# iagostorch/VVC-MIP-GPU

Measured on AMD Instinct MI355X. Metric: 1080p frames/sec, full MIP mode search over all CU sizes; 1/2/4/8 GPU, higher is better.
Workload: dtype int16x2/int32

## Files before the change

vvc-mip-gpu_amd/csrc/mip_kernels.h:

```cpp
#pragma once
#include <hip/hip_runtime.h>
#include <stdint.h>

#include "mipgpu.h"

namespace mipgpu {

struct Job {
  uint32_t cost;
  uint8_t lx, ly;
  uint16_t cu;
};
struct WaveTask {
  uint8_t cls;
  uint8_t ncu;
  uint8_t q0, q1;
  uint32_t cu0;
};

constexpr int kNumClasses = 29;
constexpr int kNumBaseClasses = 17;
constexpr int kClassW[kNumClasses] = {64, 32, 32, 16, 32, 8, 16, 16, 8, 32, 4, 16, 4, 8, 8, 4, 4, 32, 16, 16, 8,
                                      4, 4, 4, 8, 8, 8, 32, 16};
constexpr int kClassH[kNumClasses] = {64, 32, 16, 32, 8, 32, 16, 8, 16, 4, 32, 4, 16, 8, 4, 8, 4, 8, 16, 8, 16,
                                      32, 16, 8, 32, 16, 16, 16, 32};
#ifndef MIP_SIX_WAVES
#define MIP_SIX_WAVES 3
#endif
constexpr int kV16 = MIP_SIX_WAVES == 1 || MIP_SIX_WAVES == 2 ? 2 : 1;
constexpr int kClassV[kNumClasses] = {4, 2, 1, 2, 1, 1, kV16, kV16, 1, 1, 2, 1, 2, 1, 1, 1, 1, 2, 4, 2, 4,
                                      2, 2, 1, 1, 1, 4, 2, 4};
constexpr bool kClassTR[kNumClasses] = {false, false, false, false, false, false, false, false, false, false, false,
                                        false, false, false, false, false, false, false, false, false, false,
                                        true, true, true, true, true, true, false, false};
constexpr int kClassVariant[kNumClasses] = {-1, -1, 27, 28, 17, -1, 18, 19, 20, -1, -1, -1, -1, -1, -1, -1, -1,
                                            -1, -1, -1, -1, -1, -1, -1, -1, 26, -1, -1, -1};
constexpr int kClassTransposed[kNumBaseClasses] = {-1, -1, -1, -1, 24, -1, -1, 25, -1, 21, -1, 22, -1, -1, 23, -1, -1};
constexpr int size_class(int w, int h) {
  for (int i = 0; i < kNumBaseClasses; i++)
    if (kClassW[i] == w && kClassH[i] == h) return i;
  return -1;
}
constexpr int class_size_id(int w, int h) { return (w == 4 && h == 4) ? 0 : ((w == 4 || h == 4 || (w == 8 && h == 8)) ? 1 : 2); }
constexpr int class_slots(int cls) { return 64 / ((kClassW[cls] / 4) * kClassV[cls]); }

struct SearchArgs {
  const uint16_t *orig;
  const uint16_t *refs;
  int32_t *cost;
  uint8_t *best_mode;
  int32_t *best_cost;
  uint32_t *split_acc;
  const uint16_t *dfill;
  const int *dfill_begin;
  int32_t *sad;
  int32_t *satd;
  const WaveTask *tasks;
  const Job *jobs;
  const int *list_begin;
  const uint32_t *fill;
  const int *fill_begin;
  const uint8_t *ctu_var;
  const uint4 *tables;
  int width, height;
  int ctu_cols, nctus;
  int ctu0, nrange;
  int slices;
  uint32_t *queue;
  uint32_t nitems;
  const uint32_t *order;
  uint32_t nframes;
  uint32_t chunks;
  uint64_t *wave_clock;
  uint32_t *status;
  uint32_t *const *frame_status;
  int check_refs;
  uint32_t nonempty;
};
constexpr int kStatusOrig = 0, kStatusRefs = 1, kStatusWords = 4;
constexpr uint32_t kAbove10Bits = 0xfc00fc00u;
constexpr int kClockSlots = 128;
constexpr int kQueueChunks = 8;
constexpr int kQueueWords = 16;
constexpr int kMaxCtuVariants = 255;

constexpr float kAccInitS2 = 0.5f - 1024.0f;
constexpr int kWeightRows = 768, kWeightRowOffS1 = 384, kWeightRowOffS0 = 512;
constexpr int kCtabRows = 384 + 4;
constexpr int kTableBytes = kWeightRows * 16 + kCtabRows * 4;

struct FixupCu {
  uint32_t ctu;
  uint16_t cu;
  uint8_t shape;
  uint8_t pad;
};

struct BestArgs {
  const int32_t *cost;
  uint8_t *best_mode;
  int32_t *best_cost;
  int total_cus;
  int k;
};
constexpr int kMaxBestK = 32;

struct FilterArgs {
  const uint16_t *in;
  uint16_t *out;
  int width, height, nframes;
  int filter;
  int kernel_idx;
};

constexpr int kSearchWaves = MIP_SIX_WAVES == 1 || MIP_SIX_WAVES == 3 ? 12 : 8, kWideWaves = 16;
int search_resident_groups(bool alt_refs, bool wide);
#if !defined(MIP_FOUR_WAVE_TWIN) || !MIP_FOUR_WAVE_TWIN
int search_resident_groups_four(bool alt_refs, bool wide);
#endif
hipError_t launch_search(const SearchArgs &a, int nframes, bool alt_refs, int resident, bool wide, hipStream_t s,
                         hipEvent_t done = nullptr);
#if !defined(MIP_FOUR_WAVE_TWIN) || !MIP_FOUR_WAVE_TWIN
hipError_t launch_search_four(const SearchArgs &a, int nframes, bool alt_refs, int resident, bool wide, hipStream_t s,
                         hipEvent_t done = nullptr);
#endif
hipError_t launch_best_modes(const BestArgs &a, hipStream_t s);
struct SplitArgs {
  const uint16_t *split;
  const int *split_begin;
  const uint8_t *ctu_var;
  uint8_t *best_mode;
  int32_t *best_cost;
  int nctus, ctu0, nrange, max_split;
  uint32_t *acc;
};
hipError_t launch_dec_split(const SplitArgs &a, int nframes, bool init, hipStream_t s);
hipError_t launch_filter(const FilterArgs &a, hipStream_t s);
hipError_t launch_copy(const void *src, void *dst, size_t bytes, hipStream_t s);
struct CopyPiece {
  const uint8_t *src;
  uint8_t *dst;
  uint64_t bytes;
};
constexpr int kMaxCopyPieces = 64;
struct CopyPieces {
  CopyPiece p[kMaxCopyPieces];
  int n;
};
hipError_t launch_gather_copy(const CopyPieces &a, hipStream_t s);
hipError_t launch_fixup(const SearchArgs &a, const FixupCu *cus, int n, int nframes, hipStream_t s);

struct PredictArgs {
  const uint16_t *refs;
  const mip_pred_item *items;
  long long n;
  const uint8_t *unavail;
  const uint32_t *geo;
  uint16_t *out;
  long long out_samples;
  uint32_t *skipped;
  int width, height, ctu_cols, nctus, nframes;
  int refs_vec;
};
hipError_t launch_predict(const PredictArgs &a, hipStream_t s);

}
```

vvc-mip-gpu_amd/csrc/mip_search.hip:

```cpp
#include <algorithm>
#include <cstdlib>
#include <type_traits>
#include <utility>

#include <hip/hip_ext.h>

#ifndef MIP_FOUR_WAVE_TWIN
#define MIP_FOUR_WAVE_TWIN 0
#endif
#if MIP_FOUR_WAVE_TWIN
#define launch_search launch_search_four
#define search_resident_groups search_resident_groups_four
#define search_lds_bytes search_lds_bytes_four
#endif

#include "mip_kernels.h"
#include "mip_tables.h"

namespace mipgpu {
namespace {

typedef short __attribute__((ext_vector_type(2))) s2;
typedef unsigned short __attribute__((ext_vector_type(2))) u2;
typedef _Float16 __attribute__((ext_vector_type(2))) h2;
typedef _Float16 __attribute__((ext_vector_type(4))) h4;
typedef float __attribute__((ext_vector_type(4))) f4;

[[maybe_unused]] __constant__ mip_shape_desc c_shapes[MIP_NUM_SHAPES] = MIP_SHAPE_TABLE;
struct ShapeStarts {
  uint16_t v[MIP_NUM_SHAPES + 1];
};
constexpr mip_shape_desc kShapesC[MIP_NUM_SHAPES] = MIP_SHAPE_TABLE;
constexpr ShapeStarts make_shape_starts() {
  ShapeStarts st{};
  for (int i = 0; i < MIP_NUM_SHAPES; i++) st.v[i + 1] = (uint16_t)(st.v[i] + kShapesC[i].ncu);
  return st;
}
static_assert(make_shape_starts().v[MIP_NUM_SHAPES] == MIP_CUS_PER_CTU, "shape table");
[[maybe_unused]] __constant__ ShapeStarts c_shape_start = make_shape_starts();

#ifndef MIP_PREFETCH_MIN_ITEMS
#define MIP_PREFETCH_MIN_ITEMS 32
#endif
#ifndef MIP_PF_BATCH
#define MIP_PF_BATCH 10
#endif
#ifndef MIP_PHASEA_BATCH_NCS
#define MIP_PHASEA_BATCH_NCS 2
#endif
#ifndef MIP_ACC_PAIR
#define MIP_ACC_PAIR 1
#endif
#ifndef MIP_UV2_UNROLL
#define MIP_UV2_UNROLL 2
#endif
#ifndef MIP_WIN_UNROLL
#define MIP_WIN_UNROLL 2
#endif
#ifndef MIP_PAIR_BLOCKS
#define MIP_PAIR_BLOCKS 1
#endif
#ifndef MIP_PRIO_BALANCE
#define MIP_PRIO_BALANCE 0
#endif
#ifndef MIP_ONLY_CLASS
#define MIP_ONLY_CLASS -1
#endif
#ifndef MIP_SKIP_CLASSES
#define MIP_SKIP_CLASSES 0
#endif

constexpr int kPitch = 68;
constexpr int kColOff = 4;
constexpr int kTileElems = (65 * kPitch + 7) / 8 * 8;
constexpr int kLatRowPitch = kPitch, kLatColPitch = 66;
constexpr int kLatElems = (16 * kLatRowPitch + 16 * kLatColPitch + 7) / 8 * 8;
constexpr int kEntryBytes = 16;
constexpr int kCuTableBytes = 64 * kEntryBytes;
#ifndef MIP_SCRATCH_WORDS
#define MIP_SCRATCH_WORDS \
  (MIP_SIX_WAVES == 1 ? 1152 : (MIP_SIX_WAVES == 2 ? 1144 : (MIP_SIX_WAVES == 3 ? 768 : 1280)))
#endif
constexpr bool kSpanChunks = MIP_SIX_WAVES == 3;
constexpr int kScratchWords = MIP_SCRATCH_WORDS;
constexpr int kWaveBytes = kCuTableBytes + kScratchWords * 4;
constexpr int kWaveStride = kWaveBytes;
constexpr int kZeroBytes = 7 * 8 * kEntryBytes + 16;
constexpr int kUnavailable = 0x7fffffff;

constexpr uint32_t kBiasD[2][4] = {{15345, 1023, 3069, 1023}, {7161, 1023, 3069, 1023}};
constexpr uint32_t kBiasP[4] = {32736, 24552, 16368, 16368};
constexpr uint32_t kBiasQ = 8184;
constexpr uint32_t splat32(uint32_t v) { return v | v << 16; }
constexpr uint32_t bias_word(int y, int x) { return kBiasD[y & 1][x & 3] | kBiasD[y & 1][(x + 1) & 3] << 16; }

__device__ __forceinline__ int tidx(int x, int y) { return (y + 1) * kPitch + x + kColOff; }
__device__ __forceinline__ s2 as_s2(uint32_t v) { return __builtin_bit_cast(s2, v); }
__device__ __forceinline__ u2 as_u2(s2 v) { return __builtin_bit_cast(u2, v); }
__device__ __forceinline__ s2 as_s2(u2 v) { return __builtin_bit_cast(s2, v); }
__device__ __forceinline__ s2 splat(int v) { return s2{(short)v, (short)v}; }
__device__ __forceinline__ s2 smax(s2 a, s2 b) { return __builtin_elementwise_max(a, b); }

constexpr int ilog2c(int v) { return v <= 1 ? 0 : 1 + ilog2c(v / 2); }

__device__ __forceinline__ s2 avg_round(s2 a, s2 b) {
  const uint32_t t = __builtin_bit_cast(uint32_t, a) + __builtin_bit_cast(uint32_t, b) + 0x00010001u;
  return __builtin_bit_cast(s2, __builtin_bit_cast(u2, t) >> (u2){1, 1});
}

template <class F, int... I>
__device__ __forceinline__ void static_for_impl(F &f, std::integer_sequence<int, I...>) {
  (f(std::integral_constant<int, I>{}), ...);
}
template <int N, class F>
__device__ __forceinline__ void static_for(F &&f) {
  static_for_impl(f, std::make_integer_sequence<int, N>{});
}

template <int O>
__device__ __forceinline__ u2 pk_mad_c(u2 a, u2 c) {
  if constexpr (O == 1) {
    return a + c;
  } else {
    u2 d;
    asm("v_pk_mad_u16 %0, %1, %2, %3 op_sel_hi:[1,0,1]" : "=v"(d) : "v"(a), "i"(O), "v"(c));
    return d;
  }
}
template <int O, int C>
__device__ __forceinline__ u2 pk_mad_cc(u2 a) {
  u2 d;
  asm("v_pk_mad_u16 %0, %1, %2, %3 op_sel_hi:[1,0,0]" : "=v"(d) : "v"(a), "i"(O), "i"(C));
  return d;
}

__device__ __forceinline__ void wave_lds_sync() {
  __builtin_amdgcn_fence(__ATOMIC_RELEASE, "wavefront");
  __builtin_amdgcn_wave_barrier();
  __builtin_amdgcn_fence(__ATOMIC_ACQUIRE, "wavefront");
}

template <int W, int H, int VP = kClassV[size_class(W, H)]>
struct Geo {
  static constexpr int SID = class_size_id(W, H);
  static constexpr int R = SID == 2 ? 8 : 4;
  static constexpr int RBS = SID == 0 ? 2 : 4;
  static constexpr int NOUT = R * R;
  static constexpr int UH = W / R, UV = H / R;
  static constexpr int LH = ilog2c(UH), LV = ilog2c(UV);
  static constexpr int S = W / 4;
  static constexpr int V = VP;
  static constexpr int SLOTS = 64 / (S * V);
  static constexpr int KV = R / V;
  static constexpr int CROWS = UH != 1 ? (kSpanChunks && 64 / (S * V) * (R * (R + 1) + 1) > kScratchWords ? R / 2 : R)
                               : 64 / (S * V) * (NOUT + 4) <= kScratchWords ? R
                               : !kSpanChunks ? (SID == 2 ? R / 2 : R)
                               : 64 / (S * V) * (NOUT / 2 + 4) > kScratchWords ? R / 4 : R / 2;
  static constexpr bool CHUNKED = CROWS < R;
  static constexpr int NCH = R / CROWS;
  static constexpr int CPOS = CROWS * R;
  static constexpr bool PAD = UH > 1;
  static constexpr int RP = PAD ? R + 1 : R;
  static constexpr int PITCH = UH == 1 ? (SLOTS * (CPOS + 4) <= kScratchWords ? CPOS + 4 : CPOS) : CROWS * RP + 1;
  static constexpr int WBASE = SID == 2 ? 0 : (SID == 1 ? kWeightRowOffS1 : kWeightRowOffS0);
  static constexpr int MODES = SID == 2 ? 6 : (SID == 1 ? 8 : 16);
  static_assert(SLOTS * S * V == 64, "lanes");
  static_assert(SLOTS * PITCH <= kScratchWords, "scratch");
  static_assert(V == 1 || (!CHUNKED && SID != 0 && (UV >= 4 || KV % (4 / UV) == 0)), "row parts");
  static_assert(!CHUNKED || (CROWS >= 2 && (kSpanChunks || (SID == 2 && NCH == 2))), "chunks");
};

template <bool LAT>
struct RefTile {
  const uint16_t *t;
  template <int PH>
  __device__ __forceinline__ int top(int x, int y) const {
    return LAT ? t[((y + 1) >> 2) * kLatRowPitch + x + kColOff] : t[tidx(x, y)] - (int)kBiasD[1][PH];
  }
  __device__ __forceinline__ uint2 top4(int x, int y) const {
    const uint2 v = *reinterpret_cast<const uint2 *>(t + (LAT ? ((y + 1) >> 2) * kLatRowPitch + x + kColOff : tidx(x, y)));
    return LAT ? v : make_uint2(v.x - bias_word(3, 0), v.y - bias_word(3, 2));
  }
  __device__ __forceinline__ int left(int x, int y) const {
    return LAT ? t[16 * kLatRowPitch + ((x + 1) >> 2) * kLatColPitch + y + 1] : t[tidx(x, y)] - (int)kBiasD[0][3];
  }
  template <int PH>
  __device__ __forceinline__ int left_ph(int x, int y) const { return left(x, y); }
};

template <bool LAT>
struct RefTileT {
  RefTile<LAT> r;
  template <int PH>
  __device__ __forceinline__ int top(int x, int y) const { return r.left(y, x); }
  __device__ __forceinline__ uint2 top4(int x, int y) const {
    return make_uint2((uint32_t)r.left(y, x) | (uint32_t)r.left(y, x + 1) << 16,
                      (uint32_t)r.left(y, x + 2) | (uint32_t)r.left(y, x + 3) << 16);
  }
  template <int PH>
  __device__ __forceinline__ int left_ph(int x, int y) const { return r.template top<PH>(y, x); }
  __device__ __forceinline__ int left(int x, int y) const {
    const int ph = y & 3;
    return ph == 0 ? left_ph<0>(x, y) : ph == 1 ? left_ph<1>(x, y) : ph == 2 ? left_ph<2>(x, y) : left_ph<3>(x, y);
  }
};

__device__ __forceinline__ uint2 lds_row4(const uint16_t *tile, int x, int y) {
  return *reinterpret_cast<const uint2 *>(tile + tidx(x, y));
}

struct CuPos {
  int lx, ly;
  bool top, left;
  int padT, padL;
};

template <bool TR, class RT>
__device__ __forceinline__ CuPos cu_pos(const Job &j, int fx0, int fy0, const RT &rt) {
  CuPos c;
  c.lx = TR ? j.ly : j.lx;
  c.ly = TR ? j.lx : j.ly;
  c.top = (TR ? fx0 : fy0) + c.ly > 0;
  c.left = (TR ? fy0 : fx0) + c.lx > 0;
  c.padT = c.left ? rt.template left_ph<0>(c.lx - 1, c.ly) : 512;
  c.padL = c.top ? rt.template top<0>(c.lx, c.ly - 1) : 512;
  return c;
}

template <int W, int H, class RT>
__device__ __forceinline__ void write_inputs(const CuPos &c, const RT &rt, uint8_t *entry) {
  using G = Geo<W, H>;
  constexpr int dfT = W / G::RBS, l2T = ilog2c(dfT), rndT = dfT > 1 ? dfT / 2 : 0;
  constexpr int dfL = H / G::RBS, l2L = ilog2c(dfL), rndL = dfL > 1 ? dfL / 2 : 0;
  uint32_t redT[G::RBS], redL[G::RBS];
  static_for<G::RBS>([&](auto i_c) {
    constexpr int i = decltype(i_c)::value;
    uint32_t s = 0;
    if constexpr (dfT >= 4) {
#pragma unroll
      for (int t = 0; t < dfT; t += 4) {
        const uint2 v = rt.top4(c.lx + i * dfT + t, c.ly - 1);
        s += (v.x & 0xffff) + (v.x >> 16) + (v.y & 0xffff) + (v.y >> 16);
      }
    } else {
      static_for<dfT>([&](auto t_c) {
        constexpr int off = i * dfT + decltype(t_c)::value;
        s += rt.template top<off & 3>(c.lx + off, c.ly - 1);
      });
    }
    redT[i] = c.top ? (s + rndT) >> l2T : c.padT;
    uint32_t l = 0;
    static_for<dfL>([&](auto t_c) {
      constexpr int off = i * dfL + decltype(t_c)::value;
      l += rt.template left_ph<off & 3>(c.lx - 1, c.ly + off);
    });
    redL[i] = c.left ? (l + rndL) >> l2L : c.padL;
  });
  constexpr uint32_t kBias = 0x64006400u;
  uint4 e;
  if constexpr (G::RBS == 4) {
    e = make_uint4(redT[0] | redT[1] << 16, redT[2] | redT[3] << 16, redL[0] | redL[1] << 16, redL[2] | redL[3] << 16);
  } else {
    const uint32_t t01 = redT[0] | redT[1] << 16, l01 = redL[0] | redL[1] << 16;
    e = make_uint4(t01, l01, l01, t01);
  }
  e.x |= kBias;
  e.y |= kBias;
  e.z |= kBias;
  e.w |= kBias;
  *reinterpret_cast<uint4 *>(entry) = e;
}

struct BlockAcc {
  uint32_t t[16];
  uint32_t pos;
};

__device__ __forceinline__ uint32_t as_u32(s2 v) { return __builtin_bit_cast(uint32_t, v); }
__device__ __forceinline__ uint32_t as_u32(u2 v) { return __builtin_bit_cast(uint32_t, v); }
__device__ __forceinline__ u2 as_u2(uint32_t v) { return __builtin_bit_cast(u2, v); }

template <int I>
__device__ __forceinline__ void block_row(BlockAcc &b, const s2 (&prow)[4], uint2 orow) {
  constexpr const uint32_t *B = kBiasD[I & 1];
  const s2 o01 = as_s2(orow.x), o23 = as_s2(orow.y);
  const uint32_t d0 = as_u32(s2{o01.x, o01.x} - prow[0]), d1 = as_u32(s2{o01.y, o01.y} - prow[1]);
  const uint32_t d2 = as_u32(s2{o23.x, o23.x} - prow[2]), d3 = as_u32(s2{o23.y, o23.y} - prow[3]);
  const uint32_t p0 = as_u32(__builtin_elementwise_sub_sat(as_u2(d0), (u2){(unsigned short)B[0], (unsigned short)B[0]}));
  const uint32_t p1 = as_u32(__builtin_elementwise_sub_sat(as_u2(d1), (u2){(unsigned short)B[1], (unsigned short)B[1]}));
  const uint32_t p2 = as_u32(__builtin_elementwise_sub_sat(as_u2(d2), (u2){(unsigned short)B[2], (unsigned short)B[2]}));
  const uint32_t p3 = as_u32(__builtin_elementwise_sub_sat(as_u2(d3), (u2){(unsigned short)B[3], (unsigned short)B[3]}));
  b.pos = I == 0 ? p0 + p1 + p2 + p3 : b.pos + p0 + p1 + p2 + p3;
  const uint32_t s0 = d0 + d1, s1 = d0 - d1, s2_ = d2 + d3, s3 = d2 - d3;
  b.t[4 * I + 0] = s0 + s2_;
  b.t[4 * I + 1] = s1 + s3;
  b.t[4 * I + 2] = s0 - s2_;
  b.t[4 * I + 3] = s1 - s3;
}

template <uint32_t BETA>
__device__ __forceinline__ uint32_t fold_pair(uint32_t a, uint32_t b) {
  static_assert(2 * BETA < 65536, "bias");
  const u2 mx = __builtin_elementwise_max(as_u2(a), as_u2(b)), mn = __builtin_elementwise_min(as_u2(a), as_u2(b));
  const uint32_t ng = splat32(2 * BETA) - as_u32(mn);
  return as_u32(__builtin_elementwise_max(mx, as_u2(ng))) - splat32(BETA);
}

__device__ __forceinline__ void block_finish(const BlockAcc &b, u2 &sad, u2 &satd) {
  uint32_t T = 0, m0 = 0;
  s2 dc = splat(0);
  static_for<4>([&](auto c_c) {
    constexpr int c = decltype(c_c)::value;
    const uint32_t u0 = b.t[c] + b.t[4 + c], u1 = b.t[c] - b.t[4 + c];
    const uint32_t u2_ = b.t[8 + c] + b.t[12 + c], u3 = b.t[8 + c] - b.t[12 + c];
    T += fold_pair<kBiasQ>(u1, u3);
    if constexpr (c == 0) {
      m0 = fold_pair<kBiasP[0]>(u0, u2_);
      dc = as_s2(u0) - as_s2(splat32(2 * kBiasP[0]) - u2_);
    } else {
      T += fold_pair<kBiasP[c]>(u0, u2_);
    }
  });
  const s2 adc = smax(dc, splat(0) - dc);
  const uint32_t U = m0 + m0 - as_u32(adc) + as_u32(as_u2(adc) >> (u2){2, 2});
  satd = as_u2(T + as_u32(as_u2(U + 0x00010001u) >> (u2){1, 1}));
  sad = as_u2(as_s2(b.pos + b.pos) - dc);
}

struct PairAcc {
  uint32_t sad0 = 0, sad1 = 0;
  uint32_t t0 = 0, t1 = 0;
};

template <int I>
__device__ __forceinline__ void residual_row(const s2 (&prow)[4], uint2 orow, uint32_t (&d)[4]) {
  const s2 o01 = as_s2(orow.x), o23 = as_s2(orow.y);
  d[0] = as_u32(s2{o01.x, o01.x} - prow[0]);
  d[1] = as_u32(s2{o01.y, o01.y} - prow[1]);
  d[2] = as_u32(s2{o23.x, o23.x} - prow[2]);
  d[3] = as_u32(s2{o23.y, o23.y} - prow[3]);
}
// ... 70 lines not shown
    satd0 = __builtin_amdgcn_udot2(satd, (u2){1, 0}, satd0, false);
    satd1 = __builtin_amdgcn_udot2(satd, (u2){0, 1}, satd1, false);
  }
  __device__ __forceinline__ void flush() {}
#endif
};

struct PackedAcc {
  uint32_t sad = 0, satd = 0;
  __device__ __forceinline__ void add(u2 s, u2 t) {
    sad += as_u32(s);
    satd += as_u32(t);
  }
};

struct OrigT {
  uint32_t v[4];
};

struct BlockAccTr {
  uint32_t t[16];
  uint32_t pos;
};

template <int I>
__device__ __forceinline__ void residual_row(const s2 (&prow)[4], const OrigT &o, uint32_t (&d)[4]) {
#pragma unroll
  for (int c = 0; c < 4; c++) d[c] = as_u32(s2{(short)o.v[c], (short)o.v[c]} - prow[c]);
}

template <int I>
__device__ __forceinline__ void block_row(BlockAccTr &b, const s2 (&prow)[4], const OrigT &o) {
  uint32_t d[4];
  residual_row<I>(prow, o, d);
  uint32_t p = 0;
  static_for<4>([&](auto c_c) {
    constexpr int c = decltype(c_c)::value;
    constexpr unsigned short B = (unsigned short)kBiasD[c & 1][I];
    p += as_u32(__builtin_elementwise_sub_sat(as_u2(d[c]), (u2){B, B}));
    b.t[4 * I + c] = d[c];
  });
  b.pos = I == 0 ? p : b.pos + p;
}

__device__ __forceinline__ void rows_transform_tr(const uint32_t (&raw)[16], uint32_t (&t)[16]) {
#pragma unroll
  for (int r = 0; r < 4; r++) {
    const uint32_t e0 = raw[r], e1 = raw[4 + r], e2 = raw[8 + r], e3 = raw[12 + r];
    const uint32_t s0 = e0 + e1, s1 = e0 - e1, s2_ = e2 + e3, s3 = e2 - e3;
    t[4 * r + 0] = s0 + s2_;
    t[4 * r + 1] = s1 + s3;
    t[4 * r + 2] = s0 - s2_;
    t[4 * r + 3] = s1 - s3;
  }
}

__device__ __forceinline__ void block_finish(const BlockAccTr &b, u2 &sad, u2 &satd) {
  BlockAcc r;
  rows_transform_tr(b.t, r.t);
  r.pos = b.pos;
  block_finish(r, sad, satd);
}

template <int I>
__device__ __forceinline__ void pair_row_tr(const uint32_t *dA, const uint32_t (&dB)[4], uint32_t (&t0)[16],
                                            uint32_t (&t1)[16], PairAcc &acc) {
  static_for<4>([&](auto c_c) {
    constexpr int c = decltype(c_c)::value;
    const uint32_t m0 = __builtin_amdgcn_perm(dB[c], dA[c], 0x05040100u);
    const uint32_t m1 = __builtin_amdgcn_perm(dB[c], dA[c], 0x07060302u);
    acc.sad0 = __builtin_amdgcn_sad_u16(m0, splat32(kBiasD[c & 1][I]), acc.sad0);
    acc.sad1 = __builtin_amdgcn_sad_u16(m1, splat32(kBiasD[c & 1][I]), acc.sad1);
    t0[4 * I + c] = m0;
    t1[4 * I + c] = m1;
  });
}

__device__ __forceinline__ uint32_t pair_finish_tr(const uint32_t (&raw)[16], uint32_t T) {
  uint32_t t[16];
  rows_transform_tr(raw, t);
  return pair_finish(t, T);
}

template <int R, int RP = R>
struct Red {
  static constexpr int OFF = RP > R ? 1 : 0;
  const uint32_t *p;
  int k0;
  static __device__ __forceinline__ s2 clip(uint32_t v) {
    return __builtin_bit_cast(s2, __builtin_elementwise_min(__builtin_bit_cast(u2, v), (u2){1023, 1023}));
  }
  __device__ __forceinline__ s2 operator()(int k, int kx) const { return clip(p[(k + k0) * RP + kx + OFF]); }
  __device__ __forceinline__ void row4(int k, int kx, s2 (&out)[4]) const {
    static_assert(RP == R, "row4 reads unpadded rows");
    const uint4 v = *reinterpret_cast<const uint4 *>(p + (k + k0) * R + kx);
    out[0] = clip(v.x);
    out[1] = clip(v.y);
    out[2] = clip(v.z);
    out[3] = clip(v.w);
  }
};

template <int W, int H, class RED>
__device__ __forceinline__ void anchor_row(const RED &red, int k, int x0, s2 (&a)[4]) {
  using G = Geo<W, H>;
  if constexpr (G::UH == 1) {
    red.row4(k, x0, a);
  } else if constexpr (G::UH == 2) {
    const int kx = x0 >> 1;
    const s2 r0 = red(k, kx), r1 = red(k, kx + 1);
    const s2 before = red(k, kx - 1);
    a[0] = avg_round(before, r0);
    a[1] = r0;
    a[2] = avg_round(r0, r1);
    a[3] = r1;
  } else {
    const int kx = x0 >> G::LH;
    const s2 after = red(k, kx);
    const s2 before = red(k, kx - 1);
    const uint32_t delta = as_u32(after) - as_u32(before);
    const u2 base = pk_mad_cc<G::UH, G::UH / 2>(as_u2(before));
    uint32_t n = as_u32(base);
    if constexpr (G::UH == 8) {
      const u2 hdelta = as_u2(after - before);
      const uint32_t o0 = splat32(x0 & (G::UH - 1));
      u2 base0;
      asm("v_pk_mad_u16 %0, %1, %2, %3" : "=v"(base0) : "v"(hdelta), "v"(o0), "v"(base));
      n = as_u32(base0);
    }
    static_for<4>([&](auto oc) {
      constexpr int c = decltype(oc)::value;
      if constexpr (G::UH == 4 && c == 3) {
        a[c] = after;
      } else {
        n += delta;
        a[c] = as_s2(as_u2(n) >> (u2){G::LH, G::LH});
      }
    });
  }
}

template <int H>
struct OrigRows {
  static constexpr bool TR = false;
  using Block = BlockAcc;
  static constexpr bool CACHED = H <= 4;
  uint2 r[CACHED ? H : 1];
  const uint16_t *row0;
  __device__ __forceinline__ void load(const uint16_t *t, int xx, int yy) {
    row0 = t + tidx(xx, yy);
    if constexpr (CACHED) {
#pragma unroll
      for (int i = 0; i < H; i++) r[i] = lds_row4(t, xx, yy + i);
    }
  }
  __device__ __forceinline__ uint2 operator()(int i) const {
    if constexpr (CACHED) return r[i];
    else return *reinterpret_cast<const uint2 *>(row0 + i * kPitch);
  }
};

template <int H>
struct OrigRowsT {
  static constexpr bool TR = true;
  using Block = BlockAccTr;
  const uint16_t *tile;
  int x, y;
  __device__ __forceinline__ void load(const uint16_t *t, int xx, int yy) {
    tile = t;
    x = xx;
    y = yy;
  }
  __device__ __forceinline__ OrigT operator()(int i) const {
// ... 315 lines not shown
  uint8_t *wave;
  int ctu, frame;
  int fx0, fy0;
};

__device__ __forceinline__ uint32_t floor_sat(float f) { return (uint32_t)f; }

template <int W, int H, int V, bool TR>
__device__ __forceinline__ void phase_a(const Ctx &x, int lane, int ncu, int q, int chunk) {
  using G = Geo<W, H, V>;
  const int r = lane & 15, h = lane >> 4;
  const int m0 = TR ? 2 * q - G::MODES : 2 * q;
  constexpr bool HALF = G::CHUNKED && G::SID != 2;
  constexpr bool TR2 = TR && G::SID == 2 && G::CHUNKED && G::CROWS == 2;
  const int jrow = TR2 ? 8 * (r >> 1) + (r & 1) : (G::SID == 2 && TR) ? 8 * (r >> 2) + (r & 3) : r;
  const uint8_t *abase = x.w + ((G::WBASE + (m0 + (h >> 1)) * G::NOUT + jrow) * 8 + 4 * (h & 1)) * 2;
  const bool bsel = (h >> 1) == (r & 1);
  const uint8_t *bbase = bsel ? x.wave + (r >> 1) * kEntryBytes + 8 * ((h & 1) ^ (TR ? 1 : 0)) : x.zero;
  f4 cin;
  if constexpr (G::SID == 2) {
    cin = *reinterpret_cast<const f4 *>(reinterpret_cast<const float *>(x.w + kWeightRows * 16) + 384);
  } else {
    const float *ct = reinterpret_cast<const float *>(x.w + kWeightRows * 16) + (G::WBASE - kWeightRowOffS1);
    cin = *reinterpret_cast<const f4 *>(ct + (m0 + (r & 1)) * G::NOUT + 4 * h);
  }
  constexpr int NCS = (G::SLOTS + 7) / 8;
  const int ncs_run = __builtin_amdgcn_readfirstlane((ncu + 7) >> 3);
  constexpr int NRB = HALF ? 1 : G::CPOS / 16;
  constexpr int PSTEP = TR ? G::RP : 1;
  const int pos0 = TR2 ? 2 * h : TR ? h + G::PAD : (G::PAD ? (4 * h / G::R) * G::RP + (4 * h) % G::R + 1 : 4 * h);
  uint8_t *lane_dst = x.wave + kCuTableBytes + ((r >> 1) * G::PITCH + pos0) * 4 + 2 * (r & 1);
#pragma unroll
  for (int rb = 0; rb < NRB; rb++) {
    int jofs, pofs;
    if constexpr (TR2) {
      jofs = 2 * chunk;
      pofs = 0;
    } else if constexpr (G::SID == 2) {
      const int rbg = G::CHUNKED ? NRB * chunk + rb : rb;
      const int cofs = G::CHUNKED ? G::CPOS * chunk : 0;
      const int crow = G::CHUNKED ? G::CROWS * chunk * G::RP : 0;
      if constexpr (!TR) {
        jofs = 16 * rbg;
        pofs = G::PAD ? 2 * rbg * G::RP - crow : 16 * rbg - cofs;
      } else {
        const int cc = rbg >> 1, rr = rbg & 1;
        jofs = 32 * rr + 4 * cc;
        pofs = G::PAD ? 4 * cc * G::RP + 4 * rr - crow : 32 * cc + 4 * rr - cofs;
      }
    } else {
      jofs = 0;
      pofs = HALF ? -8 * chunk : 0;
    }
    const h4 av = *reinterpret_cast<const h4 *>(abase + jofs * 16);
    constexpr bool BATCH_B = NRB == 1 && NCS >= MIP_PHASEA_BATCH_NCS;
    h4 bvs[BATCH_B ? NCS : 1];
    if constexpr (BATCH_B) {
#pragma unroll
      for (int cs = 0; cs < NCS; cs++) bvs[cs] = *reinterpret_cast<const h4 *>(bbase + cs * 8 * kEntryBytes);
    }
#pragma unroll
    for (int cs = 0; cs < NCS; cs++) {
      if (cs > 0 && cs >= ncs_run) break;
      const h4 bv = BATCH_B ? bvs[BATCH_B ? cs : 0] : *reinterpret_cast<const h4 *>(bbase + cs * 8 * kEntryBytes);
      const f4 d = __builtin_amdgcn_mfma_f32_16x16x16f16(av, bv, cin, 0, 0, 0);
      if ((G::SLOTS % 8 == 0 || 8 * cs + (r >> 1) < ncu) && (!HALF || TR || (h >> 1) == chunk)) {
        uint8_t *dst = lane_dst + (pofs + 8 * cs * G::PITCH) * 4;
        static_for<4>([&](auto i_c) {
          constexpr int i = decltype(i_c)::value;
          constexpr int off = TR2 ? (i & 1) * G::R + (i >> 1) : i * PSTEP;
          if (!(HALF && TR) || (i >> 1) == chunk) {
            const uint32_t v = floor_sat(d[i]);
            *reinterpret_cast<uint16_t *>(dst + off * 4) = (uint16_t)v;
          }
        });
      }
    }
  }
}

template <int W, int H, int V, bool TR>
__device__ __forceinline__ void phase_a_half(const Ctx &x, int lane, int q, int chunk) {
  using G = Geo<W, H, V>;
  static_assert(G::CHUNKED && G::SID != 2 && G::SLOTS == 64 && G::CROWS == 2 && !G::PAD && G::PITCH >= 8, "half chunks");
  const int r = lane & 15, h = lane >> 4;
  const int m0 = TR ? 2 * q - G::MODES : 2 * q;
  auto jout = [&](int p) { return TR ? 4 * (p & 3) + 2 * chunk + (p >> 2) : 8 * chunk + p; };
  auto pos_of_row = [](int row) { return ((row >> 1) >> 1) + 4 * ((row >> 1) & 1); };
  const uint8_t *aptr = h < 2 ? x.w + ((G::WBASE + (m0 + (r & 1)) * G::NOUT + jout(pos_of_row(r))) * 8 + 4 * h) * 2
                              : x.zero;
  const h4 av = *reinterpret_cast<const h4 *>(aptr);
  const uint8_t *bbase = x.wave + r * kEntryBytes + 8 * ((h & 1) ^ (TR ? 1 : 0));
  const float *ct = reinterpret_cast<const float *>(x.w + kWeightRows * 16) + (G::WBASE - kWeightRowOffS1);
  f4 cin;
  static_for<4>([&](auto i_c) {
    constexpr int i = decltype(i_c)::value;
    cin[i] = ct[(m0 + (i & 1)) * G::NOUT + jout(h + 4 * (i >> 1))];
  });
  h4 bvs[4];
#pragma unroll
  for (int cs = 0; cs < 4; cs++) bvs[cs] = *reinterpret_cast<const h4 *>(bbase + cs * 16 * kEntryBytes);
  uint8_t *lane_dst = x.wave + kCuTableBytes + (r * G::PITCH + h) * 4;
#pragma unroll
  for (int cs = 0; cs < 4; cs++) {
    const f4 d = __builtin_amdgcn_mfma_f32_16x16x16f16(av, bvs[cs], cin, 0, 0, 0);
    uint8_t *dst = lane_dst + 16 * cs * G::PITCH * 4;
    static_for<4>([&](auto i_c) {
      constexpr int i = decltype(i_c)::value;
      typedef __attribute__((address_space(3))) volatile uint16_t lds_u16;
      *(lds_u16 *)(dst + 16 * (i >> 1) + 2 * (i & 1)) = (uint16_t)floor_sat(d[i]);
    });
  }
}

template <int W, int H, int V>
__device__ __forceinline__ void phase_a(const Ctx &x, int lane, int ncu, int q, int chunk) {
  using G = Geo<W, H, V>;
  if constexpr (G::CHUNKED && G::SID != 2) {
    if (q >= G::MODES / 2) phase_a_half<W, H, V, true>(x, lane, q, chunk);
    else phase_a_half<W, H, V, false>(x, lane, q, chunk);
  } else {
    if (q >= Geo<W, H>::MODES / 2) phase_a<W, H, V, true>(x, lane, ncu, q, chunk);
    else phase_a<W, H, V, false>(x, lane, ncu, q, chunk);
  }
}

template <int N>
__device__ __forceinline__ uint32_t group_sum(uint32_t v) {
  if constexpr (N >= 2) v += (uint32_t)__builtin_amdgcn_update_dpp(0, (int)v, 0x111, 0xf, 0xf, true);
  if constexpr (N >= 4) v += (uint32_t)__builtin_amdgcn_update_dpp(0, (int)v, 0x112, 0xf, 0xf, true);
  if constexpr (N >= 8) v += (uint32_t)__builtin_amdgcn_update_dpp(0, (int)v, 0x114, 0xf, 0xf, true);
  if constexpr (N >= 16) v += (uint32_t)__builtin_amdgcn_update_dpp(0, (int)v, 0x118, 0xf, 0xf, true);
  if constexpr (N >= 32) v += (uint32_t)__builtin_amdgcn_update_dpp(0, (int)v, 0x142, 0xa, 0xf, false);
  if constexpr (N >= 64) v += (uint32_t)__builtin_amdgcn_update_dpp(0, (int)v, 0x143, 0xc, 0xf, false);
  return v;
}

#ifndef MIP_PIN_SUMS
#define MIP_PIN_SUMS 1
#endif
__device__ __forceinline__ uint32_t pin_sum(uint32_t v) {
#if MIP_PIN_SUMS
  asm volatile("; pin" : "+v"(v));
#endif
  return v;
}

#ifndef MIP_COST_STORE_AUX
#define MIP_COST_STORE_AUX 0
#endif
struct CtuRows {
  __amdgpu_buffer_rsrc_t r;
  __device__ __forceinline__ explicit CtuRows(int32_t *ctu_block) {
    r = __builtin_amdgcn_make_buffer_rsrc(ctu_block, 0, MIP_COSTS_PER_CTU * 4, 0x00020000);
  }
  __device__ __forceinline__ void store(uint32_t cu_ofs, int mq, int v0, int v1) const {
    typedef unsigned int v2u __attribute__((ext_vector_type(2)));
    __builtin_amdgcn_raw_buffer_store_b64((v2u){(unsigned)v0, (unsigned)v1}, r, (int)cu_ofs, mq * 4, MIP_COST_STORE_AUX);
  }
};

__device__ __forceinline__ int opaque(int v) {
  asm volatile("; opaque" : "+v"(v));
  return v;
}

template <bool TR, bool LAT>
struct ViewOf {
  using type = RefTile<LAT>;
  static __device__ __forceinline__ type make(const RefTile<LAT> &r) { return r; }
};
template <bool LAT>
struct ViewOf<true, LAT> {
  using type = RefTileT<LAT>;
  static __device__ __forceinline__ type make(const RefTile<LAT> &r) { return RefTileT<LAT>{r}; }
};

template <int W, int H, int V, bool LAT, bool DEC, bool TR = false>
__device__ __forceinline__ void run_task(const Ctx &x, const RefTile<LAT> &rt_tile, const WaveTask &task, int lane_in) {
  using G = Geo<W, H, V>;
  const typename ViewOf<TR, LAT>::type rt = ViewOf<TR, LAT>::make(rt_tile);
  const int lane = opaque(lane_in);
  const SearchArgs &a = *x.a;
  const int ncu = task.ncu;
  const Job *jobs = a.jobs + task.cu0;
  const int slot = lane / (G::S * G::V), sub = lane % (G::S * G::V);
  const int v = sub / G::S, sx = sub % G::S, x0 = 4 * sx;
  const bool active = slot < ncu;
  const int cs = min(slot, ncu - 1);
  const Job job = jobs[cs];
  const CuPos c = cu_pos<TR>(job, x.fx0, x.fy0, rt);

  if (lane < ncu) {
    const Job jb = jobs[lane];
    const CuPos cj = cu_pos<TR>(jb, x.fx0, x.fy0, rt);
    write_inputs<W, H>(cj, rt, x.wave + lane * kEntryBytes);
  }
  std::conditional_t<TR, OrigRowsT<H>, OrigRows<H>> orig;
  orig.load(x.org, c.lx + x0, c.ly);
  const size_t ctu_row = ((size_t)x.frame * a.nctus + x.ctu) * MIP_COSTS_PER_CTU;
  const uint32_t cu_ofs = (uint32_t)job.cost * 4;
  const CtuRows rows_cost(a.cost ? a.cost + ctu_row : nullptr), rows_sad(a.sad ? a.sad + ctu_row : nullptr),
      rows_satd(a.satd ? a.satd + ctu_row : nullptr);
  const uint32_t *mine = reinterpret_cast<const uint32_t *>(x.wave + kCuTableBytes) + cs * G::PITCH;
  const Red<G::R, G::RP> red{mine, 0};
  s2 top[4];
  {
    const uint2 tv = rt.top4(c.lx + x0, c.ly - 1);
    const int t4[4] = {(int)(tv.x & 0xffff), (int)(tv.x >> 16), (int)(tv.y & 0xffff), (int)(tv.y >> 16)};
#pragma unroll
    for (int cc = 0; cc < 4; cc++) top[cc] = splat(c.top ? t4[cc] : c.padT);
  }
  constexpr int NLV = (G::R + G::S * G::V - 1) / (G::S * G::V);
  uint32_t lvs[G::PAD && G::CHUNKED ? NLV : 1];
  uint32_t *lcol = reinterpret_cast<uint32_t *>(x.wave + kCuTableBytes) + cs * G::PITCH;
  auto write_left = [&](int chunk) {
#pragma unroll
    for (int j = 0; j < NLV; j++) {
      const int k = sub + j * G::S * G::V;
      if (active && k < G::R && k / G::CROWS == chunk) lcol[(k - chunk * G::CROWS) * G::RP] = lvs[j];
    }
  };
  if constexpr (G::PAD && G::CHUNKED) {
#pragma unroll
    for (int j = 0; j < NLV; j++) {
      const int k = sub + j * G::S * G::V;
      const uint32_t lv = k < G::R && c.left ? rt.left(c.lx - 1, c.ly + k * G::UV + G::UV - 1) : c.padL;
      lvs[j] = lv | lv << 16;
    }
    write_left(0);
  } else if constexpr (G::PAD) {
    for (int k = sub; k < G::R; k += G::S * G::V) {
      const uint32_t lv = c.left ? rt.left(c.lx - 1, c.ly + k * G::UV + G::UV - 1) : c.padL;
      if (active) lcol[k * G::RP] = lv | lv << 16;
    }
  }
  wave_lds_sync();

  uint32_t best = 0xffffffffu;
  constexpr bool PAIRED = MIP_PAIR_BLOCKS && kPaired<W, H, V>;
#pragma unroll 1
  for (int q = task.q0; q < task.q1; q++) {
    std::conditional_t<PAIRED, PairAcc, std::conditional_t<(W * H <= 32), PackedAcc, Acc>> acc;
    s2 prev[4];
#pragma unroll
    for (int cc = 0; cc < 4; cc++) prev[cc] = top[cc];
    phase_a<W, H, V>(x, lane, ncu, q, 0);
    if constexpr (G::PAD && G::CHUNKED) {
      if (q > task.q0) write_left(0);
    }
    wave_lds_sync();
    if constexpr (kSpanChunks && G::CHUNKED) {
      auto sw = [&](int c) {
        wave_lds_sync();
        phase_a<W, H, V>(x, lane, ncu, q, c);
        if constexpr (G::PAD) write_left(c);
        wave_lds_sync();
      };
      if constexpr (G::SID == 0) {
        walk_4x4_chunked<W, H, V>(orig, red, sw, acc);
      } else {
        static_assert(PAIRED, "chunked classes walk block pairs");
        walk_pairs_chunked<W, H, V>(orig, red, x0, prev, acc, sw);
      }
    } else if constexpr (PAIRED && G::CHUNKED) {
      walk_pairs<W, H, V>(orig, red, x0, 0, prev, acc);
      wave_lds_sync();
      phase_a<W, H, V>(x, lane, ncu, q, 1);
      wave_lds_sync();
      const Red<G::R, G::RP> red_hi{mine, -4};
      walk_pairs<W, H, V>(orig, red_hi, x0, 4, prev, acc);
    } else if constexpr (PAIRED) {
      const int k0 = G::V > 1 ? v * G::KV : 0;
      if constexpr (G::V > 1) {
        if (k0 > 0) anchor_row<W, H>(red, k0 - 1, x0, prev);
      }
      walk_pairs<W, H, V>(orig, red, x0, k0, prev, acc);
    } else if constexpr (G::CHUNKED) {
      walk_strip<W, H, V>(orig, red, x0, 0, 4, prev, acc);
      wave_lds_sync();
      phase_a<W, H, V>(x, lane, ncu, q, 1);
      wave_lds_sync();
      const Red<G::R, G::RP> red_hi{mine, -4};
      walk_strip<W, H, V>(orig, red_hi, x0, 4, 8, prev, acc);
    } else if constexpr (G::SID == 0) {
      walk_strip<W, H, V>(orig, red, x0, 0, 4, prev, acc);
    } else {
      const int k0 = G::V > 1 ? v * G::KV : 0;
// ... 308 lines not shown
    if (b && s1.valid(k)) v1[k] = s1.load(k);
  }
  uint32_t bits0 = 0, bits1 = 0;
#pragma unroll
  for (int k = 0; k < N; k++) {
    if (s0.valid(k)) {
      bits0 |= v0[k].x | v0[k].y;
      s0.store(dst0, k, v0[k]);
    }
    if (b && s1.valid(k)) {
      bits1 |= v1[k].x | v1[k].y;
      s1.store(dst1, k, v1[k]);
    }
  }
  flag_above_10_bits(bits0, a, f0, kStatusOrig);
  flag_above_10_bits(bits1, a, f1, kStatusOrig);
}

template <bool DEC>
__device__ __forceinline__ void pair_loop(const SearchArgs &a, uint16_t *org_buf, const uint8_t *w, const uint8_t *zero,
                                          uint8_t *waves, uint32_t *counters, int wave, int lane) {
  const uint32_t ne = a.nonempty, npairs = (ne + 1) / 2;
  for (;;) {
    if (threadIdx.x == 0) {
      counters[0] = 0;
      counters[1] = atomicAdd(a.queue, 1u);
    }
    __syncthreads();
    const uint32_t p = counters[1];
    if (p >= npairs) break;
    const uint32_t i0 = p, i1 = ne - 1 - p;
    const bool two = i1 != i0;
    const ItemPos p0(a, i0), p1(a, i1);
    const int vq0 = a.ctu_var[p0.ctu] * 4 + p0.quad, vq1 = a.ctu_var[p1.ctu] * 4 + p1.quad;
    const int l0 = vq0 * a.slices + p0.slice, l1 = vq1 * a.slices + p1.slice;
    const int tb0 = a.list_begin[l0], n0 = a.list_begin[l0 + 1] - tb0;
    const int tb1 = a.list_begin[l1], n1 = two ? a.list_begin[l1 + 1] - tb1 : 0;
    fill_unavailable<DEC>(a, p0.frame, p0.ctu, vq0, p0.slice);
    if (two) fill_unavailable<DEC>(a, p1.frame, p1.ctu, vq1, p1.slice);
    for (uint32_t e = ne + p; e < a.nitems; e += npairs) {
      const ItemPos pe(a, e);
      fill_unavailable<DEC>(a, pe.frame, pe.ctu, a.ctu_var[pe.ctu] * 4 + pe.quad, pe.slice);
    }
    uint16_t *org0 = org_buf, *org1 = org_buf + kTileElems;
    stage_tiles2<64 * kWideWaves>(org0, a.orig + (size_t)p0.frame * a.width * a.height, p0.fx0, p0.fy0, org1,
                                  a.orig + (size_t)p1.frame * a.width * a.height, p1.fx0, p1.fy0, two, a.width,
                                  a.height, a, p0.frame, p1.frame);
    __syncthreads();
    uint64_t *clk0 = a.wave_clock ? a.wave_clock + (size_t)i0 * kClockSlots : nullptr;
    uint64_t *clk1 = a.wave_clock && two ? a.wave_clock + (size_t)i1 * kClockSlots : nullptr;
    if (clk0 && threadIdx.x == 0) {
      stamp_item_start(clk0);
      if (clk1) stamp_item_start(clk1);
    }
    const int m = n0 < n1 ? n0 : n1;
    for (;;) {
      uint32_t tn = 0;
      if (lane == 0) tn = atomicAdd(counters, 1u);
      const int t = (int)__builtin_amdgcn_readfirstlane(tn);
      if (t >= n0 + n1) break;
      const bool second = t < 2 * m ? (t & 1) != 0 : n1 > n0;
      const int k = t < 2 * m ? t >> 1 : t - m;
      const uint64_t c0 = clk0 ? __builtin_readcyclecounter() : 0;
      const WaveTask task = a.tasks[(second ? tb1 : tb0) + k];
      const Ctx x{&a, second ? org1 : org0, second ? org1 : org0, w, zero, waves + wave * kWaveStride,
                  second ? p1.ctu : p0.ctu, second ? p1.frame : p0.frame, second ? p1.fx0 : p0.fx0,
                  second ? p1.fy0 : p0.fy0};
      const RefTile<false> rt{x.ref};
      dispatch_task<false, DEC>(x, rt, task, lane);
      uint64_t *clk = second ? clk1 : clk0;
      if (clk && lane == 0) {
        if (k < kClockSlots - 3) clk[k] = __builtin_readcyclecounter() - c0;
        atomicMax(reinterpret_cast<unsigned long long *>(clk + kClockSlots - 2),
                  (unsigned long long)__builtin_amdgcn_s_memrealtime());
      }
    }
    __syncthreads();
  }
}

#ifndef MIP_WAVES_PER_EU
#define MIP_WAVES_PER_EU (MIP_SIX_WAVES ? 6 : 4)
#endif
#ifndef MIP_TABLES_GLOBAL
#define MIP_TABLES_GLOBAL 0
#endif
constexpr bool kTablesInLds = (!MIP_SIX_WAVES || MIP_SIX_WAVES == 3) && !MIP_TABLES_GLOBAL;
#ifndef MIP_S6_PF
#define MIP_S6_PF 1
#endif
#define MIP_PF_KERNEL (!MIP_SIX_WAVES || (MIP_SIX_WAVES == 3 && MIP_S6_PF))
constexpr bool kPrefetchKernel = MIP_PF_KERNEL;
template <bool ALT, bool DEC, bool PF_, int NW>
__global__ __launch_bounds__(64 * NW, NW == kWideWaves ? 4 : MIP_WAVES_PER_EU) void mip_search_kernel(SearchArgs a) {
  constexpr bool PF = PF_ && !ALT && NW == kSearchWaves && kPrefetchKernel;
  extern __shared__ __attribute__((aligned(16))) uint8_t smem[];
  uint16_t *org_buf = reinterpret_cast<uint16_t *>(smem);
  uint16_t *lattice = org_buf + kOrgTiles<ALT, PF, NW> * kTileElems;
  uint8_t *tab = smem + (kOrgTiles<ALT, PF, NW> * kTileElems + (ALT ? kLatElems : 0)) * 2;
  uint8_t *zero = tab + (kTablesInLds ? kTableBytes : 0);
  uint8_t *waves = zero + kZeroBytes;
  uint32_t *counters = reinterpret_cast<uint32_t *>(waves + NW * kWaveStride);
  const uint8_t *w = kTablesInLds ? tab : reinterpret_cast<const uint8_t *>(a.tables);

  if constexpr (kTablesInLds)
    for (int i = threadIdx.x; i < kTableBytes / 16; i += blockDim.x)
      reinterpret_cast<uint4 *>(tab)[i] = a.tables[i];
  for (int i = threadIdx.x; i < kZeroBytes / 16; i += blockDim.x)
    reinterpret_cast<uint4 *>(zero)[i] = make_uint4(0, 0, 0, 0);
  const int wave = __builtin_amdgcn_readfirstlane(threadIdx.x >> 6), lane = threadIdx.x & 63;

  if (NW == kWideWaves && !ALT && !PF && a.nonempty > 0) {
    pair_loop<DEC>(a, org_buf, w, zero, waves, counters, wave, lane);
  } else {
  if (threadIdx.x < kCounterWords) counters[threadIdx.x] = threadIdx.x == 2 && PF ? kTakeItem : 0u;
  __syncthreads();
  if (!PF) {
    if (threadIdx.x == 0) counters[2] = take_item(a, counters + 8);
    __syncthreads();
  }
  int par = 0;
  for (;;) {
    uint32_t *next_task = counters + 4 * par, *finished = next_task + 1;
    uint32_t item = next_task[2];
    bool staged = PF;
    if (PF && item == kTakeItem) {
      if (threadIdx.x == 0) next_task[3] = take_item(a, counters + 8);
      __syncthreads();
      item = next_task[3];
      staged = false;
    }
    if (item >= a.nitems) break;
    const ItemPos ip(a, item);
    const int ctu = ip.ctu, frame = ip.frame, slice = ip.slice, quad = ip.quad, fx0 = ip.fx0, fy0 = ip.fy0;
    const size_t fofs = (size_t)frame * a.width * a.height;
    const int var = a.ctu_var[ctu];
    const int vq = var * 4 + quad, list = vq * a.slices + slice;
    const int tbase = a.list_begin[list], ntasks = a.list_begin[list + 1] - tbase;
    uint16_t *org = org_buf + (PF ? par * kTileElems : 0);
    uint16_t *ref = ALT ? lattice : org;

    fill_unavailable<DEC>(a, frame, ctu, vq, slice);
    if (ntasks > 0) {
      if (!PF || !staged) {
        stage_tile<64 * NW>(org, a.orig + fofs, a.width, a.height, fx0, fy0, a, frame);
        if (ALT) stage_lattice<64 * NW>(ref, a.refs + fofs, a.width, a.height, fx0, fy0, a.check_refs != 0, a, frame);
        __syncthreads();
      }

      const Ctx x{&a, org, ref, w, zero, waves + wave * kWaveStride, ctu, frame, fx0, fy0};
      const RefTile<ALT> rt{ref};
      uint64_t *clk = a.wave_clock ? a.wave_clock + (size_t)item * kClockSlots : nullptr;
      if (clk && threadIdx.x == 0) stamp_item_start(clk);
      for (;;) {
        uint32_t tn = 0;
        if (lane == 0) tn = atomicAdd(next_task, 1u);
        const int t = (int)__builtin_amdgcn_readfirstlane(tn);
        if (t >= ntasks) break;
#if MIP_PRIO_BALANCE
        {
          const int rem4 = 4 * (ntasks - t);
          if (rem4 > 3 * ntasks) __builtin_amdgcn_s_setprio(3);
          else if (rem4 > 2 * ntasks) __builtin_amdgcn_s_setprio(2);
          else if (rem4 > ntasks) __builtin_amdgcn_s_setprio(1);
          else __builtin_amdgcn_s_setprio(0);
        }
#endif
        const uint64_t c0 = clk ? __builtin_readcyclecounter() : 0;
        const WaveTask task = a.tasks[tbase + t];
        dispatch_task<ALT, DEC>(x, rt, task, lane);
        if (clk && lane == 0 && t < kClockSlots - 3) clk[t] = __builtin_readcyclecounter() - c0;
      }
      if (clk && lane == 0) atomicMax(reinterpret_cast<unsigned long long *>(clk + kClockSlots - 2),
                                      (unsigned long long)__builtin_amdgcn_s_memrealtime());
    }
    if (PF) {
      uint32_t *nxt = counters + 4 * (par ^ 1);
      uint32_t r = 0;
      if (lane == 0) r = atomicAdd(finished, 1u);
      if (__builtin_amdgcn_readfirstlane(r) == 0) {
        uint32_t n = kTakeItem;
        if (lane == 0 && far_from_end(a, item)) n = take_item(a, counters + 8);
        const uint32_t nitem = __builtin_amdgcn_readfirstlane(n);
        if (nitem < a.nitems) {
          const ItemPos np(a, nitem);
          const uint16_t *nframe = a.orig + (size_t)np.frame * a.width * a.height;
          uint16_t *dst = org_buf + (par ^ 1) * kTileElems;
          const WindowStager<64> st(nframe, a.width, a.height, np.fx0, np.fy0, lane);
          constexpr int NL = WindowStager<64>::N, NB = MIP_PF_BATCH;
          uint32_t bits = 0;
#pragma unroll
          for (int k0 = 0; k0 < NL; k0 += NB) {
// ... 229 lines not shown
```

Baseline: 7877.

## Convert MIP phase-A MFMA outputs with packed normalized u16 conversion

Phase-A MFMA results are now converted with cvt_pknorm_u16 into packed 32-bit stores instead of four separate floor/saturate scalar u16 LDS stores. To make that exact, the input bias and accumulator init are rescaled, the size-0 bias table is prescaled while staged into LDS, and the reduced-sample clip becomes a shift. The half-zero B operand layout is also changed so A loads are unconditional and the unused half reads zeros from a shared zero region. This relies on careful float scaling to keep the results bit-exact, and it adds work to the LDS table staging.

Result: no change. 7949, median of 6 (+0.9%).

```diff
diff --git a/vvc-mip-gpu_amd/csrc/mip_kernels.h b/vvc-mip-gpu_amd/csrc/mip_kernels.h
--- a/vvc-mip-gpu_amd/csrc/mip_kernels.h
+++ b/vvc-mip-gpu_amd/csrc/mip_kernels.h
@@ -88,6 +88,8 @@
 constexpr int kWeightRows = 768, kWeightRowOffS1 = 384, kWeightRowOffS0 = 512;
 constexpr int kCtabRows = 384 + 4;
 constexpr int kTableBytes = kWeightRows * 16 + kCtabRows * 4;
+constexpr int kPkScaleLog2 = -10, kPkOffsetLog2 = -17;
+constexpr uint32_t kPkInputBias = 0x3c00;
 
 struct FixupCu {
   uint32_t ctu;
diff --git a/vvc-mip-gpu_amd/csrc/mip_search.hip b/vvc-mip-gpu_amd/csrc/mip_search.hip
--- a/vvc-mip-gpu_amd/csrc/mip_search.hip
+++ b/vvc-mip-gpu_amd/csrc/mip_search.hip
@@ -85,7 +85,7 @@
 constexpr int kScratchWords = MIP_SCRATCH_WORDS;
 constexpr int kWaveBytes = kCuTableBytes + kScratchWords * 4;
 constexpr int kWaveStride = kWaveBytes;
-constexpr int kZeroBytes = 7 * 8 * kEntryBytes + 16;
+constexpr int kZeroBytes = 7 * 8 * kEntryBytes + 16 + 16;
 constexpr int kUnavailable = 0x7fffffff;
 
 constexpr uint32_t kBiasD[2][4] = {{15345, 1023, 3069, 1023}, {7161, 1023, 3069, 1023}};
@@ -170,6 +170,28 @@
   static_assert(!CHUNKED || (CROWS >= 2 && (kSpanChunks || (SID == 2 && NCH == 2))), "chunks");
 };
 
+#ifndef MIP_PK_CONVERT
+#define MIP_PK_CONVERT 1
+#endif
+#ifndef MIP_HALF_ZERO_B
+#define MIP_HALF_ZERO_B 1
+#endif
+#ifndef MIP_DENSE_8XH
+#define MIP_DENSE_8XH 0
+#endif
+template <int W, int H, int V>
+constexpr bool kHalfA = Geo<W, H, V>::CHUNKED &&
+                        (Geo<W, H, V>::SID != 2 || (MIP_DENSE_8XH && MIP_PK_CONVERT && kSpanChunks && Geo<W, H, V>::UH == 1 &&
+                                                    Geo<W, H, V>::CROWS == 2 && Geo<W, H, V>::SLOTS % 16 == 0));
+template <int W, int H, int V>
+constexpr bool kPackedA = MIP_PK_CONVERT && kHalfA<W, H, V>;
+#ifndef MIP_TABLES_GLOBAL
+#define MIP_TABLES_GLOBAL 0
+#endif
+constexpr bool kTablesInLds = (!MIP_SIX_WAVES || MIP_SIX_WAVES == 3) && !MIP_TABLES_GLOBAL;
+constexpr bool kPkStagedS0 = kPackedA<4, 4, 1> && kTablesInLds;
+constexpr float kPkScale = 1.0f / (float)(1 << -kPkScaleLog2), kPkOffset = 1.0f / (float)(1 << -kPkOffsetLog2);
+
 template <bool LAT>
 struct RefTile {
   const uint16_t *t;
@@ -227,7 +249,7 @@
   return c;
 }
 
-template <int W, int H, class RT>
+template <int W, int H, bool PK, class RT>
 __device__ __forceinline__ void write_inputs(const CuPos &c, const RT &rt, uint8_t *entry) {
   using G = Geo<W, H>;
   constexpr int dfT = W / G::RBS, l2T = ilog2c(dfT), rndT = dfT > 1 ? dfT / 2 : 0;
@@ -256,7 +278,7 @@
     });
     redL[i] = c.left ? (l + rndL) >> l2L : c.padL;
   });
-  constexpr uint32_t kBias = 0x64006400u;
+  constexpr uint32_t kBias = PK ? splat32(kPkInputBias) : 0x64006400u;
   uint4 e;
   if constexpr (G::RBS == 4) {
     e = make_uint4(redT[0] | redT[1] << 16, redT[2] | redT[3] << 16, redL[0] | redL[1] << 16, redL[2] | redL[3] << 16);
@@ -493,13 +515,14 @@
   return pair_finish(t, T);
 }
 
-template <int R, int RP = R>
+template <int R, int RP = R, bool PK = false>
 struct Red {
   static constexpr int OFF = RP > R ? 1 : 0;
   const uint32_t *p;
   int k0;
   static __device__ __forceinline__ s2 clip(uint32_t v) {
-    return __builtin_bit_cast(s2, __builtin_elementwise_min(__builtin_bit_cast(u2, v), (u2){1023, 1023}));
+    if constexpr (PK) return __builtin_bit_cast(s2, __builtin_bit_cast(u2, v) >> (u2){6, 6});
+    else return __builtin_bit_cast(s2, __builtin_elementwise_min(__builtin_bit_cast(u2, v), (u2){1023, 1023}));
   }
   __device__ __forceinline__ s2 operator()(int k, int kx) const { return clip(p[(k + k0) * RP + kx + OFF]); }
   __device__ __forceinline__ void row4(int k, int kx, s2 (&out)[4]) const {
@@ -981,41 +1004,65 @@
 template <int W, int H, int V, bool TR>
 __device__ __forceinline__ void phase_a_half(const Ctx &x, int lane, int q, int chunk) {
   using G = Geo<W, H, V>;
-  static_assert(G::CHUNKED && G::SID != 2 && G::SLOTS == 64 && G::CROWS == 2 && !G::PAD && G::PITCH >= 8, "half chunks");
+  static_assert(kHalfA<W, H, V> && G::SLOTS % 16 == 0 && G::CROWS == 2 && !G::PAD && G::PITCH >= G::CPOS, "half chunks");
+  constexpr bool PK = kPackedA<W, H, V>;
+  static_assert(PK || G::SID != 2, "the 8xH chunks exist in the packed form only");
+  constexpr int NRB = G::CPOS / 8, NCS = G::SLOTS / 16;
   const int r = lane & 15, h = lane >> 4;
   const int m0 = TR ? 2 * q - G::MODES : 2 * q;
-  auto jout = [&](int p) { return TR ? 4 * (p & 3) + 2 * chunk + (p >> 2) : 8 * chunk + p; };
+  auto jout = [&](int p) { return TR ? G::R * (p % G::R) + 2 * chunk + p / G::R : G::CPOS * chunk + p; };
   auto pos_of_row = [](int row) { return ((row >> 1) >> 1) + 4 * ((row >> 1) & 1); };
+#if MIP_HALF_ZERO_B
+  const uint8_t *aptr = x.w + ((G::WBASE + (m0 + (r & 1)) * G::NOUT + jout(pos_of_row(r))) * 8 + 4 * (h & 1)) * 2;
+  const uint8_t *bbase = h < 2 ? x.wave + r * kEntryBytes + 8 * ((h & 1) ^ (TR ? 1 : 0)) : x.zero;
+#else
   const uint8_t *aptr = h < 2 ? x.w + ((G::WBASE + (m0 + (r & 1)) * G::NOUT + jout(pos_of_row(r))) * 8 + 4 * h) * 2
                               : x.zero;
-  const h4 av = *reinterpret_cast<const h4 *>(aptr);
   const uint8_t *bbase = x.wave + r * kEntryBytes + 8 * ((h & 1) ^ (TR ? 1 : 0));
-  const float *ct = reinterpret_cast<const float *>(x.w + kWeightRows * 16) + (G::WBASE - kWeightRowOffS1);
+#endif
+  constexpr int kRbStep = (TR ? 1 : 8) * 16;
+  h4 av[NRB];
+#pragma unroll
+  for (int rb = 0; rb < NRB; rb++) av[rb] = *reinterpret_cast<const h4 *>(aptr + rb * kRbStep);
+  static_assert((NCS - 1) * 16 * kEntryBytes + 8 <= kZeroBytes - 16, "zero B operands");
   f4 cin;
-  static_for<4>([&](auto i_c) {
-    constexpr int i = decltype(i_c)::value;
-    cin[i] = ct[(m0 + (i & 1)) * G::NOUT + jout(h + 4 * (i >> 1))];
-  });
-  h4 bvs[4];
-#pragma unroll
-  for (int cs = 0; cs < 4; cs++) bvs[cs] = *reinterpret_cast<const h4 *>(bbase + cs * 16 * kEntryBytes);
-  uint8_t *lane_dst = x.wave + kCuTableBytes + (r * G::PITCH + h) * 4;
-#pragma unroll
-  for (int cs = 0; cs < 4; cs++) {
-    const f4 d = __builtin_amdgcn_mfma_f32_16x16x16f16(av, bvs[cs], cin, 0, 0, 0);
-    uint8_t *dst = lane_dst + 16 * cs * G::PITCH * 4;
+  if constexpr (G::SID == 2) {
+    cin = *reinterpret_cast<const f4 *>(x.zero + kZeroBytes - 16);
+  } else {
+    static_assert(NRB == 1, "one block of C rows");
+    const float *ct = reinterpret_cast<const float *>(x.w + kWeightRows * 16) + (G::WBASE - kWeightRowOffS1);
     static_for<4>([&](auto i_c) {
       constexpr int i = decltype(i_c)::value;
-      typedef __attribute__((address_space(3))) volatile uint16_t lds_u16;
-      *(lds_u16 *)(dst + 16 * (i >> 1) + 2 * (i & 1)) = (uint16_t)floor_sat(d[i]);
+      cin[i] = ct[(m0 + (i & 1)) * G::NOUT + jout(h + 4 * (i >> 1))];
+      if constexpr (PK && !(G::SID == 0 && kPkStagedS0)) cin[i] = __builtin_fmaf(cin[i], kPkScale, kPkOffset);
     });
+  }
+  h4 bvs[NCS];
+#pragma unroll
+  for (int cs = 0; cs < NCS; cs++) bvs[cs] = *reinterpret_cast<const h4 *>(bbase + cs * 16 * kEntryBytes);
+  uint8_t *lane_dst = x.wave + kCuTableBytes + (r * G::PITCH + h) * 4;
+#pragma unroll
+  for (int it = 0; it < NRB * NCS; it++) {
+    const int rb = it / NCS, cs = it % NCS;
+    const f4 d = __builtin_amdgcn_mfma_f32_16x16x16f16(av[rb], bvs[cs], cin, 0, 0, 0);
+    uint8_t *dst = lane_dst + (16 * cs * G::PITCH + 8 * rb) * 4;
+    if constexpr (PK) {
+      *reinterpret_cast<uint32_t *>(dst) = __builtin_bit_cast(uint32_t, __builtin_amdgcn_cvt_pknorm_u16(d[0], d[1]));
+      *reinterpret_cast<uint32_t *>(dst + 16) = __builtin_bit_cast(uint32_t, __builtin_amdgcn_cvt_pknorm_u16(d[2], d[3]));
+    } else {
+      static_for<4>([&](auto i_c) {
+        constexpr int i = decltype(i_c)::value;
+        typedef __attribute__((address_space(3))) volatile uint16_t lds_u16;
+        *(lds_u16 *)(dst + 16 * (i >> 1) + 2 * (i & 1)) = (uint16_t)floor_sat(d[i]);
+      });
+    }
   }
 }
 
 template <int W, int H, int V>
 __device__ __forceinline__ void phase_a(const Ctx &x, int lane, int ncu, int q, int chunk) {
   using G = Geo<W, H, V>;
-  if constexpr (G::CHUNKED && G::SID != 2) {
+  if constexpr (kHalfA<W, H, V>) {
     if (q >= G::MODES / 2) phase_a_half<W, H, V, true>(x, lane, q, chunk);
     else phase_a_half<W, H, V, false>(x, lane, q, chunk);
   } else {
@@ -1093,7 +1140,7 @@
   if (lane < ncu) {
     const Job jb = jobs[lane];
     const CuPos cj = cu_pos<TR>(jb, x.fx0, x.fy0, rt);
-    write_inputs<W, H>(cj, rt, x.wave + lane * kEntryBytes);
+    write_inputs<W, H, kPackedA<W, H, V>>(cj, rt, x.wave + lane * kEntryBytes);
   }
   std::conditional_t<TR, OrigRowsT<H>, OrigRows<H>> orig;
   orig.load(x.org, c.lx + x0, c.ly);
@@ -1102,7 +1149,7 @@
   const CtuRows rows_cost(a.cost ? a.cost + ctu_row : nullptr), rows_sad(a.sad ? a.sad + ctu_row : nullptr),
       rows_satd(a.satd ? a.satd + ctu_row : nullptr);
   const uint32_t *mine = reinterpret_cast<const uint32_t *>(x.wave + kCuTableBytes) + cs * G::PITCH;
-  const Red<G::R, G::RP> red{mine, 0};
+  const Red<G::R, G::RP, kPackedA<W, H, V>> red{mine, 0};
   s2 top[4];
   {
     const uint2 tv = rt.top4(c.lx + x0, c.ly - 1);
@@ -1577,10 +1624,6 @@
 #ifndef MIP_WAVES_PER_EU
 #define MIP_WAVES_PER_EU (MIP_SIX_WAVES ? 6 : 4)
 #endif
-#ifndef MIP_TABLES_GLOBAL
-#define MIP_TABLES_GLOBAL 0
-#endif
-constexpr bool kTablesInLds = (!MIP_SIX_WAVES || MIP_SIX_WAVES == 3) && !MIP_TABLES_GLOBAL;
 #ifndef MIP_S6_PF
 #define MIP_S6_PF 1
 #endif
@@ -1599,10 +1642,23 @@
   const uint8_t *w = kTablesInLds ? tab : reinterpret_cast<const uint8_t *>(a.tables);
 
   if constexpr (kTablesInLds)
-    for (int i = threadIdx.x; i < kTableBytes / 16; i += blockDim.x)
-      reinterpret_cast<uint4 *>(tab)[i] = a.tables[i];
-  for (int i = threadIdx.x; i < kZeroBytes / 16; i += blockDim.x)
-    reinterpret_cast<uint4 *>(zero)[i] = make_uint4(0, 0, 0, 0);
+    for (int i = threadIdx.x; i < kTableBytes / 16; i += blockDim.x) {
+      uint4 v = a.tables[i];
+      if constexpr (kPkStagedS0) {
+        constexpr int c0 = kWeightRows + (kWeightRowOffS0 - kWeightRowOffS1) / 4;
+        if (i >= c0 && i < c0 + (kWeightRows - kWeightRowOffS0) / 4) {
+          auto sc = [](uint32_t u) {
+            return __builtin_bit_cast(uint32_t, __builtin_fmaf(__builtin_bit_cast(float, u), kPkScale, kPkOffset));
+          };
+          v = make_uint4(sc(v.x), sc(v.y), sc(v.z), sc(v.w));
+        }
+      }
+      reinterpret_cast<uint4 *>(tab)[i] = v;
+    }
+  for (int i = threadIdx.x; i < kZeroBytes / 16; i += blockDim.x) {
+    const uint32_t c = i == kZeroBytes / 16 - 1 ? __builtin_bit_cast(uint32_t, kAccInitS2 * kPkScale + kPkOffset) : 0u;
+    reinterpret_cast<uint4 *>(zero)[i] = make_uint4(c, c, c, c);
+  }
   const int wave = __builtin_amdgcn_readfirstlane(threadIdx.x >> 6), lane = threadIdx.x & 63;
 
   if (NW == kWideWaves && !ALT && !PF && a.nonempty > 0) {
```
